# strasdat/ScaViSLAM

Hardware: AMD Instinct MI355X
Metric: stereo frames/sec + DWO Schur ms @ 50 KF / 20k pts (higher is better)
Workload: dtype u8/int32 (FAST, ZNSSD), f32+f64 (dense tracking), f64 (Schur); 1 GPU

## Files before the change

scavislam_amd/csrc/common.h:

```cpp
#pragma once
#include <hip/hip_runtime.h>
#include <stdint.h>
#include <stdio.h>
#include <memory>
#include <string>

#include "../../include/scavislam_hip.h"
#include "owned.h"
#include "devutil.h"

struct svs_ctx {
  int device = 0;
  int n_cu = 256;
  hipStream_t stream = nullptr;
  owned::Stream own_stream;
  owned::Event ev0, ev1;
  std::string err;
  DevBuf<void> scratch;
  DevBuf<void> match_scratch;
  int trk_nwg = 0;
  int trk_balance = 1;
  int trk_regs = 0;
  int full_nwg = 0;
  int match_legacy = 0;
  int mo_spec = 1;
  int fe_fuse_tail = 1;
  int match_order = 1;
  int fe_pipeline = 1;
  int fe_overlap = 1;
  int trk_seq_chi2 = 0;
  int trk_lazy_chi2 = 1;
  int trk_split = 10;
  int trk_cont_slots = 0;
  const double *match_src_T = nullptr, *match_src_Ta = nullptr;
  DevBuf<void> seq_buf;
  DevBuf<unsigned> seq_stats;
  owned::Event spin_ev;
  owned::Event lane_ev;
  bool spin_lane = false;
  int spin_demand = 0;
  long long spin_n_lane = 0, spin_n_gated = 0;
  long long stereo_n_prefilter16 = 0, stereo_n_prefilter4 = 0, stereo_n_strip_filter = 0, stereo_n_frame_filter = 0, stereo_n_validate_wide = 0, stereo_n_strips = 0;
  DevBuf<int> stereo_err;
  int xcd_swizzle = 1;
  float vocab_ms[3] = {0.f, 0.f, 0.f};
  int mo_legacy = 0;
  long long stereo_n_wide_search = 0;
};
int svs_spin_enter(svs_ctx *ctx, int n_workgroups = 0);
int svs_spin_leave(svs_ctx *ctx);
struct SvsSpinScope {
  svs_ctx *ctx; int rc; bool open;
  SvsSpinScope(svs_ctx *c, int n_workgroups = 0) : ctx(c), rc(svs_spin_enter(c, n_workgroups)), open(rc == 0) {}
  int leave() { if (!open) return SVS_OK; open = false; return svs_spin_leave(ctx); }
  ~SvsSpinScope() { if (open) (void)svs_spin_leave(ctx); }
  SvsSpinScope(const SvsSpinScope &) = delete;
  SvsSpinScope &operator=(const SvsSpinScope &) = delete;
};
int svs_ctx_grow(svs_ctx *ctx, DevBuf<void> svs_ctx::*which, size_t bytes, void **out);
inline int svs_ctx_scratch(svs_ctx *ctx, size_t bytes, void **out) { return svs_ctx_grow(ctx, &svs_ctx::scratch, bytes, out); }
inline int svs_ctx_match_scratch(svs_ctx *ctx, size_t bytes, void **out) { return svs_ctx_grow(ctx, &svs_ctx::match_scratch, bytes, out); }
size_t svs_dense_track_balance_bytes(int batch);
const int *svs_dense_track_balance_order(svs_ctx *ctx, void *d_bal_state, int batch);
int svs_dense_track_balance_init(svs_ctx *ctx, void *d_bal_state, int batch);
int svs_dense_track_cpu_sem_work(svs_ctx *ctx, const svs_dense_track_args *a, double *d_T_io, int32_t *d_passes_out, int batch, void *d_bal_state);
#define SVS_DEVICE(ctx) SVS_HIP(ctx, hipSetDevice((ctx)->device))

#define SVS_HIP(ctx, call)                                                              \
  do {                                                                                  \
    hipError_t e_ = (call);                                                             \
    if (e_ != hipSuccess) {                                                             \
      char buf_[512];                                                                   \
      snprintf(buf_, sizeof buf_, "%s:%d %s -> %s", __FILE__, __LINE__, #call,          \
               hipGetErrorString(e_));                                                  \
      (ctx)->err = buf_;                                                                \
      return SVS_ERR_HIP;                                                               \
    }                                                                                   \
  } while (0)

#define SVS_REQUIRE(ctx, cond)                                                          \
  do {                                                                                  \
    if (!(cond)) {                                                                      \
      char buf_[512];                                                                   \
      snprintf(buf_, sizeof buf_, "%s:%d requirement failed: %s", __FILE__, __LINE__,   \
               #cond);                                                                  \
      if (ctx) (ctx)->err = buf_;                                                       \
      return SVS_ERR_INVALID;                                                           \
    }                                                                                   \
  } while (0)

#define SVS_LAUNCH_CHECK(ctx) SVS_HIP(ctx, hipGetLastError())

int svs_pyr_down_u8_copy(svs_ctx *ctx, const uint8_t *d_src, int w, int h, int sstride, size_t s_bstride, uint8_t *d_dst, int dstride, size_t d_bstride,
                         uint8_t *d_copy, int cstride, size_t c_bstride, int batch);
struct svs_mo_tail {
  const svs_candidate_point *pts; size_t pts_b; const int32_t *n_new; float mre; svs_gated_point *gated; size_t gated_b; svs_point_stats *ptstats;
  const float *disp; int ds; size_t disp_b; svs_cam cams[3]; float *cloud[3]; size_t cloud_b[3];
  const int *order;
};
int svs_motion_only_gate_cloud(svs_ctx *ctx, const svs_match_result *d_results, int n, size_t res_bstride, const svs_cam *cam, const svs_pose_opt_params *prm,
                               double *d_T_io, svs_pose_opt_stats *d_stats, const svs_mo_tail *tail, int batch);
int svs_process_matched_points_dev(svs_ctx *ctx, const svs_match_result *d_results, const svs_candidate_point *d_pts, int n, size_t res_bstride,
                                   size_t pts_bstride, const int32_t *d_n_new_records, const svs_cam *cam, const double *d_T, float max_reproj_error,
                                   svs_gated_point *d_gated, size_t gated_bstride, svs_point_stats *d_stats, int batch);

int svs_pointcloud_cpu_sem_levels(svs_ctx *ctx, const float *d_disp, int disp_stride, size_t disp_bstride, const svs_cam *cams, const double *d_T, float *const *d_cloud,
                                  const size_t *cloud_bstride, int batch);

struct svs_loop;
int svs_loop_set_place_dev(svs_loop *l, int slot, int n, const float *d_desc, const double *d_uvu);
svs_ctx *svs_loop_ctx(svs_loop *l);
```

scavislam_amd/csrc/fast.hip:

```cpp
#include "common.h"
#include "fast_view.h"
#include <algorithm>
#include <cstdlib>
#include <vector>

namespace {

struct LevelDev {
  int w, h;
  int gx, gy, cell_w, cell_h;
  int min_inner, min_outer, max_inner, max_outer, fast_min, fast_max;
  int cell_base;
  uint32_t *bm;
  int bm_wpr, bm_stride;
  size_t bm_bstride;
  int16_t *xy;
};
struct FastParams {
  LevelDev lv[SVS_NUM_PYR_LEVELS];
  int n_levels, ncell_total, cap, t_lo;
  unsigned *hist;
  int *thr, *emit, *count, *offset;
  int *level_total;
  uint32_t *cand; int *cand_n;
  int *cell_tile0, *cell_ntile;
  int n_tiles;
  int swz;
};
constexpr int CAND_CAP = 2048;
constexpr int BM_LDS_MAX = 144 * 1024;
struct ImgPtrs {
  const uint8_t *img[SVS_NUM_PYR_LEVELS];
  int stride[SVS_NUM_PYR_LEVELS];
  size_t bstride[SVS_NUM_PYR_LEVELS];
};
struct TileDesc { int16_t level, cell, x0, y0; };

constexpr int TW = 64, TH = 32, HALO = 3;

__device__ __constant__ int8_t c_ring_dx[16] = {0, 1, 2, 3, 3, 3, 2, 1, 0, -1, -2, -3, -3, -3, -2, -1};
__device__ __constant__ int8_t c_ring_dy[16] = {3, 3, 2, 1, 0, -1, -2, -3, -3, -3, -2, -1, 0, 1, 2, 3};

__device__ __forceinline__ int arc9_maxmin(const int (&d)[16]) {
  int m2[16], m4[16], best = -1024;
#pragma unroll
  for (int k = 0; k < 16; ++k) m2[k] = min(d[k], d[(k + 1) & 15]);
#pragma unroll
  for (int k = 0; k < 16; ++k) m4[k] = min(m2[k], m2[(k + 2) & 15]);
#pragma unroll
  for (int k = 0; k < 16; ++k) {
    int m8 = min(m4[k], m4[(k + 4) & 15]);
    int m9 = min(m8, d[(k + 8) & 15]);
    best = max(best, m9);
  }
  return best;
}

typedef short s16x2 __attribute__((ext_vector_type(2)));
__device__ __forceinline__ s16x2 as_s16x2(uint32_t u) { s16x2 r; __builtin_memcpy(&r, &u, 4); return r; }
__device__ __forceinline__ s16x2 arc9_maxmin_pk(const s16x2 (&d)[16]) {
  s16x2 m2[16], m4[16], best = {-1024, -1024};
#pragma unroll
  for (int k = 0; k < 16; ++k) m2[k] = __builtin_elementwise_min(d[k], d[(k + 1) & 15]);
#pragma unroll
  for (int k = 0; k < 16; ++k) m4[k] = __builtin_elementwise_min(m2[k], m2[(k + 2) & 15]);
#pragma unroll
  for (int k = 0; k < 16; ++k) {
    const s16x2 m8 = __builtin_elementwise_min(m4[k], m4[(k + 4) & 15]);
    const s16x2 m9 = __builtin_elementwise_min(m8, d[(k + 8) & 15]);
    best = __builtin_elementwise_max(best, m9);
  }
  return best;
}

constexpr int LROW = 19;
__device__ __forceinline__ int byte_of(const uint32_t (&w)[3], int b) { return (w[b >> 2] >> (8 * (b & 3))) & 0xff; }
__device__ __forceinline__ uint32_t pair_of(const uint32_t (&w)[3], int b) {
  const int j = b >> 2, j1 = (j + 1 < 3) ? j + 1 : j;
  const unsigned i0 = (unsigned)(b & 3);
  const unsigned i1 = ((b + 1) >> 2) == j ? (unsigned)((b + 1) & 3) : 4u + (unsigned)((b + 1) & 3);
  return __builtin_amdgcn_perm(w[j1], w[j], i0 | (0x0cu << 8) | (i1 << 16) | (0x0cu << 24));
}

__global__ __launch_bounds__(256, 8) void fast_score_kernel(FastParams P, ImgPtrs I, const TileDesc *__restrict__ tiles) {
  __shared__ uint32_t s_img[(TH + 2 * HALO) * LROW];
  __shared__ unsigned s_hist[256];
  __shared__ uint16_t s_surv[TW * TH];
  __shared__ int s_ncorn, s_nsurv;
  unsigned wg = blockIdx.y * gridDim.x + blockIdx.x;
  if (P.swz) wg = xcd_contiguous(wg, gridDim.x * gridDim.y);
  const int tile_i = wg % gridDim.x, slot = wg / gridDim.x;
  const TileDesc td = tiles[tile_i];
  const LevelDev &L = P.lv[td.level];
  const int tid = threadIdx.x;
  const int ci = td.cell % L.gx, cj = td.cell / L.gx;
  const int u0 = ci * L.cell_w, v0 = cj * L.cell_h;
  const uint8_t *img = I.img[td.level] + (size_t)slot * I.bstride[td.level];
  const int istride = I.stride[td.level];
  s_hist[tid] = 0;
  const int gx0 = u0 + td.x0 - 4, gy0 = v0 + td.y0 - HALO;
  for (int i = tid; i < (TH + 2 * HALO) * 18; i += 256) {
    const int r = i / 18, c = i - r * 18;
    const int y = min(max(gy0 + r, 0), L.h - 1), x = gx0 + 4 * c;
    const uint8_t *row = img + (size_t)y * istride;
    const int xs = min(max(x, 0), L.w - 4), d = x - xs;
    uint32_t raw;
    __builtin_memcpy(&raw, row + xs, 4);
    const uint32_t v = d == 0 ? raw : d >= 4 || d <= -4 ? 0u : d > 0 ? raw >> (8 * d) : raw << (-8 * d);
    s_img[r * LROW + c] = v;
  }
  __syncthreads();
  const int tx = tid & 15;
  const int cx0 = td.x0 + 4 * tx;
  if (tid == 0) { s_ncorn = 0; s_nsurv = 0; }
  __syncthreads();
  const int t = P.t_lo;
  constexpr int RDX[16] = {0, 1, 2, 3, 3, 3, 2, 1, 0, -1, -2, -3, -3, -3, -2, -1};
  constexpr int RDY[16] = {3, 3, 2, 1, 0, -1, -2, -3, -3, -3, -2, -1, 0, 1, 2, 3};
#pragma unroll 1
  for (int ty = tid >> 4; ty < TH; ty += 16) {
    const int cy = td.y0 + ty;
    uint32_t win[7][3];
#pragma unroll
    for (int r = 0; r < 7; r += 3)
#pragma unroll
      for (int c = 0; c < 3; ++c) win[r][c] = s_img[(ty + r) * LROW + tx + c];
    const bool row_ok = cy >= 3 && cy < L.cell_h - 3;
    const uint32_t Kd = 0x7fff7fffu - (uint32_t)t * 0x00010001u;
#pragma unroll
    for (int p = 0; p < 2; ++p) {
      const uint32_t vpair = pair_of(win[3], 4 + 2 * p);
      const uint32_t Vd = vpair + Kd, Vb = Kd - vpair;
      uint32_t X[4], Y[4];
#pragma unroll
      for (int i = 0; i < 4; ++i) {
        const int q = 4 * i;
        const uint32_t rp = pair_of(win[3 + RDY[q]], 4 + 2 * p + RDX[q]);
        X[i] = Vd - rp; Y[i] = rp + Vb;
      }
      const uint32_t pass = ((X[0] & X[1]) | (X[1] & X[2]) | (X[2] & X[3]) | (X[3] & X[0]) | (Y[0] & Y[1]) | (Y[1] & Y[2]) | (Y[2] & Y[3]) | (Y[3] & Y[0])) & 0x80008000u;
#pragma unroll
      for (int h = 0; h < 2; ++h) {
        const int k = 2 * p + h, cx = cx0 + k;
        const bool surv = row_ok && cx >= 3 && cx < L.cell_w - 3 && ((pass >> (16 * h)) & 0x8000u) != 0;
        if (surv) { const int slot_i = atomicAdd(&s_nsurv, 1); s_surv[slot_i] = (uint16_t)((ty << 8) | (4 * tx + k)); }
      }
    }
  }
  __syncthreads();
  const int nsurv = s_nsurv;
  const uint8_t *s_b8 = reinterpret_cast<const uint8_t *>(s_img);
  uint32_t *cand = P.cand + ((size_t)slot * P.n_tiles + tile_i) * CAND_CAP;
  for (int i = tid; i < nsurv; i += 256) {
    const int code = s_surv[i], py = code >> 8, px = code & 0xff;
    const int cb = (py + 3) * (LROW * 4) + px + 4;
    const int v = s_b8[cb];
    s16x2 d[16];
#pragma unroll
    for (int q = 0; q < 16; ++q) {
      const int r = s_b8[cb + RDY[q] * (LROW * 4) + RDX[q]];
      const int x = v - r;
      d[q] = as_s16x2(((uint32_t)x & 0xffffu) | ((uint32_t)(-x) << 16));
    }
    const s16x2 b2 = arc9_maxmin_pk(d);
    const int sc = max((int)b2.x, (int)b2.y) - 1;
    if (sc >= t) {
      const int s8 = min(sc + 1, 255);
      atomicAdd(&s_hist[s8], 1u);
      cand[atomicAdd(&s_ncorn, 1)] = ((uint32_t)s8 << 24) | ((uint32_t)(td.y0 + py) << 12) | (uint32_t)(td.x0 + px);
    }
  }
  __syncthreads();
  if (tid == 0) P.cand_n[(size_t)slot * P.n_tiles + tile_i] = s_ncorn;
  const unsigned c = s_hist[tid];
  if (c) atomicAdd(&P.hist[((size_t)slot * P.ncell_total + L.cell_base + td.cell) * 256 + tid], c);
}

__global__ __launch_bounds__(256) void fast_adapt_kernel(FastParams P, int trials) {
  extern __shared__ int s_cnt[];
  const int slot = blockIdx.x;
  const int tid = threadIdx.x, lane = tid & 63, wave = tid >> 6;
  unsigned *hist = P.hist + (size_t)slot * P.ncell_total * 256;
  for (int c = wave; c < P.ncell_total; c += 4) {
    uint4 hv = *reinterpret_cast<const uint4 *>(hist + (size_t)c * 256 + 4 * lane);
    *reinterpret_cast<uint4 *>(hist + (size_t)c * 256 + 4 * lane) = make_uint4(0, 0, 0, 0);
    int a3 = hv.w, a2 = hv.z + a3, a1 = hv.y + a2, a0 = hv.x + a1;
    int tot = a0, run = tot;
#pragma unroll
    for (int o = 1; o < 64; o <<= 1) { int up = __shfl_down(run, o, 64); if (lane + o < 64) run += up; }
    int above = run - tot;
    s_cnt[c * 256 + 4 * lane + 0] = a0 + above;
    s_cnt[c * 256 + 4 * lane + 1] = a1 + above;
    s_cnt[c * 256 + 4 * lane + 2] = a2 + above;
    s_cnt[c * 256 + 4 * lane + 3] = a3 + above;
  }
  __syncthreads();
  int *thr = P.thr + (size_t)slot * P.ncell_total;
  int *emit = P.emit + (size_t)slot * P.ncell_total;
  int *count = P.count + (size_t)slot * P.ncell_total;
  int *offset = P.offset + (size_t)slot * P.ncell_total;
  int row = tid, lvl = -1, j = 0;
  for (int l = 0; l < P.n_levels; ++l) { if (row < P.lv[l].gy) { lvl = l; j = row; break; } row -= P.lv[l].gy; }
  if (lvl >= 0) {
    const LevelDev &L = P.lv[lvl];
    int prev_thr = -1, prev_prev_thr = -2;
    for (int i = 0; i < L.gx; ++i) {
      const int c = L.cell_base + j * L.gx + i;
      int t = thr[c], used = t, num = 0;
      if (trials <= 0) {
        int tc = min(max(t, 0), 255);
        num = tc + 1 <= 255 ? s_cnt[c * 256 + tc + 1] : 0;
      }
      for (int trial = 0; trial < trials; ++trial) {
        used = t;
        int tc = min(max(t, 0), 255);
        num = tc + 1 <= 255 ? s_cnt[c * 256 + tc + 1] : 0;
        if (prev_prev_thr == t) { t = (t + prev_prev_thr) / 2; break; }
        prev_prev_thr = prev_thr;
        prev_thr = t;
        if (num < L.min_inner) {
          if (t <= L.fast_min) break;
          --t;
          if (num < L.min_outer) { if (t <= L.fast_min) break; --t; continue; }
        } else if (num > L.max_inner) {
          if (t >= L.fast_max) break;
          ++t;
          if (num > L.max_outer) { if (t >= L.fast_max) break; ++t; continue; }
        }
        break;
      }
      thr[c] = t; emit[c] = used; count[c] = num;
    }
  }
  __syncthreads();
  if (tid < P.n_levels) {
    const LevelDev &L = P.lv[tid];
    int run = 0;
    for (int c = L.cell_base; c < L.cell_base + L.gx * L.gy; ++c) { offset[c] = run; run += count[c]; }
    P.level_total[(size_t)slot * P.n_levels + tid] = run;
  }
}

template <int NT>
__global__ __launch_bounds__(NT) void fast_compact_bitmap_kernel(FastParams P) {
  extern __shared__ uint32_t s_bm[];
  const int slot = blockIdx.y, c = blockIdx.x, tid = threadIdx.x, lane = tid & 63, wave = tid >> 6;
  int lvl = 0;
  while (lvl + 1 < P.n_levels && c >= P.lv[lvl + 1].cell_base) ++lvl;
  const LevelDev &L = P.lv[lvl];
  const int cl = c - L.cell_base, ci = cl % L.gx, cj = cl / L.gx;
  const int u0 = ci * L.cell_w, v0 = cj * L.cell_h;
  const int rows = L.cell_h, wpr = L.bm_wpr;
  int *s_row = reinterpret_cast<int *>(s_bm + rows * wpr);
  const int thr1 = min(max(P.emit[(size_t)slot * P.ncell_total + c], 0), 255) + 1;
  const int base = P.offset[(size_t)slot * P.ncell_total + c];
  for (int i = tid; i < rows * wpr; i += NT) s_bm[i] = 0u;
  __syncthreads();
  if (thr1 <= 255) {
    const int t0 = P.cell_tile0[c], nt = P.cell_ntile[c];
    for (int t = wave; t < nt; t += NT / 64) {
      const int n = min(P.cand_n[(size_t)slot * P.n_tiles + t0 + t], CAND_CAP);
      const uint32_t *cand = P.cand + ((size_t)slot * P.n_tiles + t0 + t) * CAND_CAP;
      for (int i = lane; i < n; i += 64) {
        const uint32_t r = cand[i];
        if ((int)(r >> 24) >= thr1) {
          const int x = r & 0xfffu, y = (r >> 12) & 0xfffu;
          atomicOr(&s_bm[y * wpr + (x >> 5)], 1u << (x & 31));
        }
      }
    }
  }
  __syncthreads();
  for (int r = tid; r < rows; r += NT) {
    int n = 0;
    for (int j = 0; j < wpr; ++j) n += __popc(s_bm[r * wpr + j]);
    s_row[r] = n;
  }
  __syncthreads();
  if (wave == 0) {
    int carry = 0;
    for (int r0 = 0; r0 < rows; r0 += 64) {
      const int v = r0 + lane < rows ? s_row[r0 + lane] : 0;
      int run = v;
#pragma unroll
      for (int o = 1; o < 64; o <<= 1) { const int dn = __shfl_up(run, o, 64); if (lane >= o) run += dn; }
      if (r0 + lane < rows) s_row[r0 + lane] = carry + run - v;
      carry += __shfl(run, 63, 64);
    }
  }
  __syncthreads();
  int16_t *xy = L.xy + (size_t)slot * P.cap * 2;
  uint32_t *gbm = L.bm + (size_t)slot * (L.bm_bstride / 4) + (size_t)v0 * (L.bm_stride / 4) + ci * wpr;
  for (int i = tid; i < rows * wpr; i += NT) {
    const int r = i / wpr, j = i - r * wpr;
    uint32_t w = s_bm[i];
    gbm[(size_t)r * (L.bm_stride / 4) + j] = w;
    if (w) {
      int pos = base + s_row[r];
      for (int k = 0; k < j; ++k) pos += __popc(s_bm[r * wpr + k]);
      while (w) {
        const int b = __ffs((int)w) - 1;
        w &= w - 1;
        if (pos < P.cap) {
          const uint32_t pk = (uint32_t)(uint16_t)(u0 + 32 * j + b) | ((uint32_t)(uint16_t)(v0 + r) << 16);
          __builtin_memcpy(xy + 2 * pos, &pk, 4);
        }
        ++pos;
      }
    }
  }
}

}

struct svs_fast {
  svs_ctx *ctx;
  FastParams P;
  int batch;
  TileDesc *d_tiles; int n_tiles;
  DevBuf<uint32_t> bm[SVS_NUM_PYR_LEVELS], cand;
  DevBuf<int16_t> xy[SVS_NUM_PYR_LEVELS];
  DevBuf<unsigned> hist;
  DevBuf<int> thr, emit, count, offset, level_total, cand_n, cell_tile0, cell_ntile;
  DevBuf<TileDesc> tiles;
  ~svs_fast() { (void)hipStreamSynchronize(ctx->stream); }
  size_t cmp_lds = 0;
};

extern "C" int svs_fast_create(svs_ctx *ctx, int n_levels, const int32_t *w, const int32_t *h,
                               const svs_fastgrid *grids, int batch, int cap, svs_fast **out) {
  SVS_REQUIRE(ctx, ctx && out && w && h && grids && n_levels >= 1 && n_levels <= SVS_NUM_PYR_LEVELS && batch >= 1 && cap >= 1);
  SVS_DEVICE(ctx);
  {
    int nc = 0;
    for (int l = 0; l < n_levels; ++l) {
      const svs_fastgrid &g = grids[l];
      SVS_REQUIRE(ctx, g.gx >= 1 && g.gy >= 1 && g.gx * g.gy <= SVS_MAX_CELLS && g.cell_w >= 1 && g.cell_h >= 1 && g.cell_w * g.gx <= w[l] && g.cell_h * g.gy <= h[l]);
      SVS_REQUIRE(ctx, g.cell_w <= 4096 && g.cell_h <= 4096);
      SVS_REQUIRE(ctx, ((size_t)g.cell_h * ((g.cell_w + 31) / 32) + g.cell_h) * 4 <= (size_t)BM_LDS_MAX);
      nc += g.gx * g.gy;
    }
    SVS_REQUIRE(ctx, (size_t)nc * 256 * 4 <= 64 * 1024);
  }
  std::unique_ptr<svs_fast> f(new svs_fast());
  f->ctx = ctx; f->batch = batch;
  FastParams &P = f->P;
  P = FastParams{};
  P.n_levels = n_levels; P.cap = cap;
  std::vector<TileDesc> tiles;
  std::vector<int> cell_tile0, cell_ntile;
  int cell_base = 0, t_lo = 255;
  for (int l = 0; l < n_levels; ++l) {
    const svs_fastgrid &g = grids[l];
    LevelDev &L = P.lv[l];
    L.w = w[l]; L.h = h[l]; L.gx = g.gx; L.gy = g.gy; L.cell_w = g.cell_w; L.cell_h = g.cell_h;
    L.min_inner = g.min_inner; L.min_outer = g.min_outer; L.max_inner = g.max_inner; L.max_outer = g.max_outer;
    L.fast_min = g.fast_min; L.fast_max = g.fast_max; L.cell_base = cell_base;
    L.bm_wpr = (g.cell_w + 31) / 32;
    const int gap = 32 * L.bm_wpr - g.cell_w;
    L.bm_stride = ((std::max(w[l], g.gx * g.cell_w) + gap * (g.gx - 1) + 7) / 8 + 8 + 15) / 16 * 16;
    SVS_REQUIRE(ctx, L.bm_stride >= 4 * L.bm_wpr * g.gx);
    L.bm_bstride = (size_t)L.bm_stride * h[l] + 16;
    SVS_HIP(ctx, f->bm[l].alloc_bytes(L.bm_bstride * batch, &L.bm));
    SVS_HIP(ctx, hipMemsetAsync(L.bm, 0, L.bm_bstride * batch, ctx->stream));
    f->cmp_lds = std::max(f->cmp_lds, ((size_t)g.cell_h * L.bm_wpr + g.cell_h) * 4);
    SVS_HIP(ctx, f->xy[l].alloc(2 * (size_t)cap * batch, &L.xy));
    for (int c = 0; c < g.gx * g.gy; ++c) {
      t_lo = std::min(t_lo, std::min(g.fast_min, g.thr[c]));
      cell_tile0.push_back((int)tiles.size());
      for (int y0 = 0; y0 < g.cell_h; y0 += TH)
        for (int x0 = 0; x0 < g.cell_w; x0 += TW) tiles.push_back(TileDesc{(int16_t)l, (int16_t)c, (int16_t)x0, (int16_t)y0});
      cell_ntile.push_back((int)tiles.size() - cell_tile0.back());
    }
    cell_base += g.gx * g.gy;
  }
  P.ncell_total = cell_base;
  P.t_lo = std::max(t_lo, 0);
  if (f->cmp_lds > 64 * 1024) {
    SVS_HIP(ctx, hipFuncSetAttribute(reinterpret_cast<const void *>(&fast_compact_bitmap_kernel<256>), hipFuncAttributeMaxDynamicSharedMemorySize, (int)f->cmp_lds));
    SVS_HIP(ctx, hipFuncSetAttribute(reinterpret_cast<const void *>(&fast_compact_bitmap_kernel<1024>), hipFuncAttributeMaxDynamicSharedMemorySize, (int)f->cmp_lds));
  }
  size_t nc = (size_t)P.ncell_total * batch;
  SVS_HIP(ctx, f->hist.alloc(nc * 256, &P.hist));
  SVS_HIP(ctx, hipMemsetAsync(P.hist, 0, nc * 256 * sizeof(unsigned), ctx->stream));
  SVS_HIP(ctx, f->thr.alloc(nc, &P.thr));
  SVS_HIP(ctx, f->emit.alloc(nc, &P.emit));
  SVS_HIP(ctx, f->count.alloc(nc, &P.count));
  SVS_HIP(ctx, f->offset.alloc(nc, &P.offset));
  SVS_HIP(ctx, f->level_total.alloc((size_t)batch * n_levels, &P.level_total));
  SVS_HIP(ctx, hipMemsetAsync(P.emit, 0, nc * sizeof(int), ctx->stream));
  SVS_HIP(ctx, hipMemsetAsync(P.count, 0, nc * sizeof(int), ctx->stream));
  SVS_HIP(ctx, hipMemsetAsync(P.offset, 0, nc * sizeof(int), ctx->stream));
  SVS_HIP(ctx, hipMemsetAsync(P.level_total, 0, (size_t)batch * n_levels * sizeof(int), ctx->stream));
  std::vector<int> thr0(nc);
  for (int b = 0; b < batch; ++b)
    for (int l = 0; l < n_levels; ++l)
      for (int c = 0; c < grids[l].gx * grids[l].gy; ++c) thr0[(size_t)b * P.ncell_total + P.lv[l].cell_base + c] = grids[l].thr[c];
  SVS_HIP(ctx, hipMemcpyAsync(P.thr, thr0.data(), nc * sizeof(int), hipMemcpyHostToDevice, ctx->stream));
  f->n_tiles = (int)tiles.size();
  P.n_tiles = f->n_tiles;
  SVS_HIP(ctx, f->cand.alloc((size_t)batch * tiles.size() * CAND_CAP, &P.cand));
  SVS_HIP(ctx, f->cand_n.alloc((size_t)batch * tiles.size(), &P.cand_n));
  SVS_HIP(ctx, f->cell_tile0.alloc(cell_tile0.size(), &P.cell_tile0));
  SVS_HIP(ctx, f->cell_ntile.alloc(cell_ntile.size(), &P.cell_ntile));
  SVS_HIP(ctx, hipMemcpyAsync(P.cell_tile0, cell_tile0.data(), sizeof(int) * cell_tile0.size(), hipMemcpyHostToDevice, ctx->stream));
  SVS_HIP(ctx, hipMemcpyAsync(P.cell_ntile, cell_ntile.data(), sizeof(int) * cell_ntile.size(), hipMemcpyHostToDevice, ctx->stream));
  SVS_HIP(ctx, f->tiles.alloc(tiles.size(), &f->d_tiles));
  SVS_HIP(ctx, hipMemcpyAsync(f->d_tiles, tiles.data(), sizeof(TileDesc) * tiles.size(), hipMemcpyHostToDevice, ctx->stream));
  SVS_HIP(ctx, hipStreamSynchronize(ctx->stream));
  *out = f.release();
  return SVS_OK;
}

extern "C" int svs_fast_destroy(svs_fast *f) {
  if (!f) return SVS_OK;
  delete f;
  return SVS_OK;
}

extern "C" int svs_fast_detect(svs_fast *f, const uint8_t *const *d_img, const int32_t *stride, const size_t *bstride,
                               int n_batch, int trials) {
  SVS_REQUIRE(f ? f->ctx : nullptr, f && d_img && stride && bstride && n_batch >= 1 && n_batch <= f->batch && trials >= 0);
  SVS_DEVICE(f->ctx);
  svs_ctx *ctx = f->ctx;
  ImgPtrs I{};
  for (int l = 0; l < f->P.n_levels; ++l) { I.img[l] = d_img[l]; I.stride[l] = stride[l]; I.bstride[l] = bstride[l]; }
  f->P.swz = ctx->xcd_swizzle;
  hipLaunchKernelGGL(fast_score_kernel, dim3(f->n_tiles, n_batch), dim3(256), 0, ctx->stream, f->P, I, f->d_tiles);
  SVS_LAUNCH_CHECK(ctx);
  hipLaunchKernelGGL(fast_adapt_kernel, dim3(n_batch), dim3(256), (size_t)f->P.ncell_total * 256 * sizeof(int), ctx->stream, f->P, trials);
  SVS_LAUNCH_CHECK(ctx);
  if ((long)f->P.ncell_total * n_batch <= 1024) hipLaunchKernelGGL(fast_compact_bitmap_kernel<1024>, dim3(f->P.ncell_total, n_batch), dim3(1024), f->cmp_lds, ctx->stream, f->P);
  else hipLaunchKernelGGL(fast_compact_bitmap_kernel<256>, dim3(f->P.ncell_total, n_batch), dim3(256), f->cmp_lds, ctx->stream, f->P);
  SVS_LAUNCH_CHECK(ctx);
  return SVS_OK;
}

extern "C" int svs_fast_download(svs_fast *f, int slot, int level, int16_t *h_xy, int cap, int32_t *h_n,
                                 int32_t *h_cell_count, int32_t *h_emit_thr, int32_t *h_thr_state) {
  SVS_REQUIRE(f ? f->ctx : nullptr, f && slot >= 0 && slot < f->batch && level >= 0 && level < f->P.n_levels);
  SVS_DEVICE(f->ctx);
  svs_ctx *ctx = f->ctx;
  const FastParams &P = f->P;
  const LevelDev &L = P.lv[level];
  int total = 0;
  SVS_HIP(ctx, hipMemcpyAsync(&total, P.level_total + (size_t)slot * P.n_levels + level, sizeof(int), hipMemcpyDeviceToHost, ctx->stream));
  SVS_HIP(ctx, hipStreamSynchronize(ctx->stream));
  if (h_n) *h_n = total;
  int nc = L.gx * L.gy;
  size_t co = (size_t)slot * P.ncell_total + L.cell_base;
  if (h_cell_count) SVS_HIP(ctx, hipMemcpyAsync(h_cell_count, P.count + co, nc * sizeof(int), hipMemcpyDeviceToHost, ctx->stream));
  if (h_emit_thr) SVS_HIP(ctx, hipMemcpyAsync(h_emit_thr, P.emit + co, nc * sizeof(int), hipMemcpyDeviceToHost, ctx->stream));
  if (h_thr_state) SVS_HIP(ctx, hipMemcpyAsync(h_thr_state, P.thr + co, nc * sizeof(int), hipMemcpyDeviceToHost, ctx->stream));
  int ncopy = std::min(std::min(total, cap), P.cap);
  if (h_xy && ncopy > 0)
    SVS_HIP(ctx, hipMemcpyAsync(h_xy, L.xy + (size_t)slot * P.cap * 2, sizeof(int16_t) * 2 * (size_t)ncopy, hipMemcpyDeviceToHost, ctx->stream));
  SVS_HIP(ctx, hipStreamSynchronize(ctx->stream));
  if (h_xy && (total > cap || total > P.cap)) return SVS_ERR_CAPACITY;
  return SVS_OK;
}

extern "C" int svs_fast_set_thresholds(svs_fast *f, int slot, int level, const int32_t *h_thr) {
  SVS_REQUIRE(f ? f->ctx : nullptr, f && h_thr && slot >= 0 && slot < f->batch && level >= 0 && level < f->P.n_levels);
  SVS_DEVICE(f->ctx);
  svs_ctx *ctx = f->ctx;
  const LevelDev &L = f->P.lv[level];
  int nc = L.gx * L.gy;
  for (int c = 0; c < nc; ++c) SVS_REQUIRE(ctx, h_thr[c] >= f->P.t_lo);
  SVS_HIP(ctx, hipMemcpyAsync(f->P.thr + (size_t)slot * f->P.ncell_total + L.cell_base, h_thr, nc * sizeof(int), hipMemcpyHostToDevice, ctx->stream));
  SVS_HIP(ctx, hipStreamSynchronize(ctx->stream));
  return SVS_OK;
}

extern "C" int svs_fast_device_view(svs_fast *f, int level, const uint32_t **d_corner_bits, int32_t *row_stride_bytes, size_t *batch_stride_bytes,
                                    int32_t *cell_column_bits, const int32_t **d_emit_thr, size_t *emit_bstride) {
  SVS_REQUIRE(f ? f->ctx : nullptr, f && level >= 0 && level < f->P.n_levels);
  const LevelDev &L = f->P.lv[level];
  if (d_corner_bits) *d_corner_bits = L.bm;
  if (row_stride_bytes) *row_stride_bytes = L.bm_stride;
  if (batch_stride_bytes) *batch_stride_bytes = L.bm_bstride;
  if (cell_column_bits) *cell_column_bits = 32 * L.bm_wpr;
  if (d_emit_thr) *d_emit_thr = f->P.emit + L.cell_base;
  if (emit_bstride) *emit_bstride = (size_t)f->P.ncell_total;
  return SVS_OK;
}

FastView svs_fast_view_internal(const svs_fast *f) {
  FastView v{};
  v.n_levels = f->P.n_levels; v.emit = f->P.emit; v.ncell_total = f->P.ncell_total;
  for (int l = 0; l < f->P.n_levels; ++l) {
    const LevelDev &L = f->P.lv[l];
    v.bm[l] = reinterpret_cast<const uint8_t *>(L.bm); v.bm_stride[l] = L.bm_stride; v.bm_bstride[l] = L.bm_bstride; v.bm_gap[l] = 32 * L.bm_wpr - L.cell_w;
    v.cell_base[l] = L.cell_base; v.gx[l] = L.gx; v.gy[l] = L.gy; v.cell_w[l] = L.cell_w; v.cell_h[l] = L.cell_h;
    v.w[l] = L.w; v.h[l] = L.h;
  }
  return v;
}

FastThrView svs_fast_thr_view_internal(svs_fast *f) {
  FastThrView v{};
  v.thr = f->P.thr; v.ncell_total = f->P.ncell_total; v.t_lo = f->P.t_lo; v.n_levels = f->P.n_levels; v.batch = f->batch;
  for (int l = 0; l < f->P.n_levels; ++l) { v.cell_base[l] = f->P.lv[l].cell_base; v.ncell[l] = f->P.lv[l].gx * f->P.lv[l].gy; }
  return v;
}

FastListView svs_fast_list_view_internal(const svs_fast *f) {
  FastListView v{};
  v.n_levels = f->P.n_levels; v.batch = f->batch; v.cap = f->P.cap; v.level_total = f->P.level_total; v.count = f->P.count; v.ncell_total = f->P.ncell_total;
  for (int l = 0; l < f->P.n_levels; ++l) { v.xy[l] = f->P.lv[l].xy; v.cell_base[l] = f->P.lv[l].cell_base; v.ncell[l] = f->P.lv[l].gx * f->P.lv[l].gy; }
  return v;
}
```

scavislam_amd/csrc/image.hip:

```cpp
#include "common.h"
#include <algorithm>
#include <mutex>
#include <vector>
#include <stdlib.h>

namespace {
struct SpinLane { svs_ctx *c; hipEvent_t ev; int cus; };
struct SpinGate { std::mutex m; hipEvent_t last = nullptr; svs_ctx *owner = nullptr; int last_cus = 0; std::vector<SpinLane> lanes; };
SpinGate g_spin_gate[64];
SpinGate &gate_of(const svs_ctx *c) { return g_spin_gate[(unsigned)c->device % 64u]; }
}
constexpr int SVS_SPIN_SMALL = 16;
int svs_spin_enter(svs_ctx *c, int n_workgroups) {
  SpinGate &g = gate_of(c);
  const int demand = n_workgroups > 0 ? std::min(n_workgroups, c->n_cu) : c->n_cu;
  g.m.lock();
  for (size_t i = 0; i < g.lanes.size();) {
    if (g.lanes[i].c != c && hipEventQuery(g.lanes[i].ev) == hipErrorNotReady) ++i;
    else if (g.lanes[i].c == c) ++i;
    else { g.lanes[i] = g.lanes.back(); g.lanes.pop_back(); }
  }
  int lanes_busy = 0;
  for (const SpinLane &l : g.lanes) if (l.c != c) lanes_busy += l.cus;
  const bool gated_busy = g.last && g.owner != c && hipEventQuery(g.last) == hipErrorNotReady;
  (void)hipGetLastError();
  c->spin_demand = demand;
  c->spin_lane = n_workgroups > 0 && n_workgroups <= SVS_SPIN_SMALL && demand + lanes_busy + (gated_busy ? g.last_cus : 0) <= c->n_cu;
  if (c->spin_lane) { ++c->spin_n_lane; return SVS_OK; }
  ++c->spin_n_gated;
  hipError_t e = hipSuccess;
  if (g.last && g.owner != c) e = hipStreamWaitEvent(c->stream, g.last, 0);
  if (demand + lanes_busy > c->n_cu)
    for (const SpinLane &l : g.lanes) if (l.c != c && e == hipSuccess) e = hipStreamWaitEvent(c->stream, l.ev, 0);
  if (e != hipSuccess) { g.m.unlock(); c->err = std::string("svs_spin_enter: hipStreamWaitEvent -> ") + hipGetErrorString(e); return SVS_ERR_HIP; }
  return SVS_OK;
}
int svs_spin_leave(svs_ctx *c) {
  SpinGate &g = gate_of(c);
  hipError_t e = hipSuccess;
  owned::Event &ev = c->spin_lane ? c->lane_ev : c->spin_ev;
  if (!ev) e = ev.create(hipEventDisableTiming);
  if (e == hipSuccess) e = hipEventRecord(ev, c->stream);
  if (e == hipSuccess) {
    if (c->spin_lane) {
      bool found = false;
      for (SpinLane &l : g.lanes) if (l.c == c) { l.ev = ev; l.cus = c->spin_demand; found = true; }
      if (!found) g.lanes.push_back(SpinLane{c, ev, c->spin_demand});
    } else { g.last = ev; g.owner = c; g.last_cus = c->spin_demand; }
  }
  c->spin_lane = false;
  g.m.unlock();
  if (e != hipSuccess) { c->err = std::string("svs_spin_leave: ") + hipGetErrorString(e); return SVS_ERR_HIP; }
  return SVS_OK;
}
static void spin_forget(svs_ctx *c) {
  SpinGate &g = gate_of(c);
  std::lock_guard<std::mutex> lk(g.m);
  for (size_t i = 0; i < g.lanes.size();) { if (g.lanes[i].c == c) { g.lanes[i] = g.lanes.back(); g.lanes.pop_back(); } else ++i; }
  if (g.owner == c) { g.last = nullptr; g.owner = nullptr; g.last_cus = 0; }
}
extern "C" int svs_ctx_create(int device, void *hip_stream, svs_ctx **out) {
  if (!out) return SVS_ERR_INVALID;
  int n = 0;
  if (hipGetDeviceCount(&n) != hipSuccess || n <= 0 || device < 0 || device >= n) return SVS_ERR_NO_DEVICE;
  std::unique_ptr<svs_ctx> c(new svs_ctx());
  c->device = device;
  if (hipSetDevice(device) != hipSuccess) return SVS_ERR_NO_DEVICE;
  { int cu = 0; if (hipDeviceGetAttribute(&cu, hipDeviceAttributeMultiprocessorCount, device) == hipSuccess && cu > 0) c->n_cu = cu; }
  if (hip_stream) c->stream = (hipStream_t)hip_stream;
  else if (c->own_stream.create(hipStreamNonBlocking) != hipSuccess) return SVS_ERR_HIP;
  else c->stream = c->own_stream;
  if (c->ev0.create() != hipSuccess || c->ev1.create() != hipSuccess) return SVS_ERR_HIP;
  if (c->stereo_err.alloc(32) != hipSuccess || hipMemset(c->stereo_err, 0, 32 * sizeof(int)) != hipSuccess) return SVS_ERR_HIP;
  auto env_int = [](const char *name, int lo, int hi) { const char *e = getenv(name); if (!e) return 0; const int v = atoi(e); return v < lo ? lo : (v > hi ? hi : v); };
  c->trk_nwg = env_int("SVS_TRK_NWG", 1, 64);
  if (const char *e = getenv("SVS_TRK_BALANCE")) { const int v = atoi(e); c->trk_balance = v < 0 || v > 1 ? 1 : v; }
  c->trk_regs = getenv("SVS_TRK_ONE_PER_CU") ? 1 : (getenv("SVS_TRK_TWO_PER_CU") ? 2 : 0);
  c->full_nwg = env_int("SVS_FULL_NWG", 1, 1024);
  *out = c.release();
  return SVS_OK;
}
extern "C" int svs_ctx_destroy(svs_ctx *c) {
  if (!c) return SVS_OK;
  (void)hipStreamSynchronize(c->stream);
  spin_forget(c);
  delete c;
  return SVS_OK;
}
int svs_ctx_grow(svs_ctx *c, DevBuf<void> svs_ctx::*which, size_t bytes, void **out) {
  SVS_REQUIRE(c, c && out);
  DevBuf<void> &buf = c->*which;
  if (buf.bytes() < bytes) {
    SVS_DEVICE(c);
    if (buf) SVS_HIP(c, hipStreamSynchronize(c->stream));
    SVS_HIP(c, buf.reserve(bytes, bytes + bytes / 2 + 4096));
  }
  *out = buf;
  return SVS_OK;
}
extern "C" int svs_ctx_set_option(svs_ctx *c, const char *name, int value) {
  SVS_REQUIRE(c, c && name && value >= 0);
  const std::string n(name);
  if (n == "trk_nwg") c->trk_nwg = value > 64 ? 64 : value;
  else if (n == "trk_regs") c->trk_regs = value > 2 ? 0 : value;
  else if (n == "trk_balance") c->trk_balance = value > 1 ? 1 : value;
  else if (n == "full_nwg") c->full_nwg = value > 1024 ? 1024 : value;
  else if (n == "mo_legacy") c->mo_legacy = value != 0;
  else if (n == "match_legacy") c->match_legacy = (int)value;
  else if (n == "fe_overlap") c->fe_overlap = value != 0;
  else if (n == "fe_pipeline") c->fe_pipeline = value != 0;
  else if (n == "match_order") c->match_order = value != 0;
  else if (n == "fe_fuse_tail") c->fe_fuse_tail = value != 0;
  else if (n == "mo_spec") c->mo_spec = value != 0;
  else if (n == "xcd_swizzle") c->xcd_swizzle = value != 0;
  else if (n == "trk_split") c->trk_split = value > 15 ? 15 : value;
  else if (n == "trk_cont_slots") c->trk_cont_slots = value > 4096 ? 4096 : value;
  else if (n == "trk_seq_chi2") c->trk_seq_chi2 = value != 0;
  else if (n == "trk_lazy_chi2") c->trk_lazy_chi2 = value > 2 ? 1 : value;
  else SVS_REQUIRE(c, !"unknown option");
  return SVS_OK;
}
extern "C" int svs_ctx_get_stat(svs_ctx *c, const char *name, long long *out) {
  SVS_REQUIRE(c, c && name && out);
  const std::string n(name);
  if (n == "spin_lane_launches") { *out = c->spin_n_lane; return SVS_OK; }
  if (n == "spin_gated_launches") { *out = c->spin_n_gated; return SVS_OK; }
  if (n == "live_device_bytes") { *out = owned::g_live_device_bytes; return SVS_OK; }
  if (n == "live_pinned_bytes") { *out = owned::g_live_pinned_bytes; return SVS_OK; }
  if (n == "live_sync_objects") { *out = owned::g_live_sync_objects; return SVS_OK; }
  if (n == "stereo_prefilter16_calls") { *out = c->stereo_n_prefilter16; return SVS_OK; }
  if (n == "stereo_prefilter4_calls") { *out = c->stereo_n_prefilter4; return SVS_OK; }
  if (n == "stereo_strip_filter_calls") { *out = c->stereo_n_strip_filter; return SVS_OK; }
  if (n == "stereo_strip_filter_strips") { *out = c->stereo_n_strips; return SVS_OK; }
  if (n == "stereo_frame_filter_calls") { *out = c->stereo_n_frame_filter; return SVS_OK; }
  if (n == "stereo_validate_wide_calls") { *out = c->stereo_n_validate_wide; return SVS_OK; }
  if (n == "stereo_wide_search_calls") { *out = c->stereo_n_wide_search; return SVS_OK; }
  if (n == "stereo_speckle_error_mask") {
    int m = 0;
    SVS_DEVICE(c);
    SVS_HIP(c, hipMemcpyAsync(&m, c->stereo_err, sizeof m, hipMemcpyDeviceToHost, c->stream));
    SVS_HIP(c, hipStreamSynchronize(c->stream));
    *out = m;
    return SVS_OK;
  }
  SVS_REQUIRE(c, n == "trk_exact_sums" || n == "trk_exact_fallbacks");
  unsigned v[2] = {0, 0};
  if (c->seq_stats) {
    SVS_DEVICE(c);
    SVS_HIP(c, hipMemcpyAsync(v, c->seq_stats, sizeof v, hipMemcpyDeviceToHost, c->stream));
    SVS_HIP(c, hipStreamSynchronize(c->stream));
  }
  *out = n == "trk_exact_sums" ? v[0] : v[1];
  return SVS_OK;
}
extern "C" int svs_api_version(void) { return SVS_API_VERSION; }
extern "C" void svs_pose_opt_params_default(svs_pose_opt_params *p) {
  if (!p) return;
  __builtin_memset(p, 0, sizeof *p);
  p->robust_kernel = 1; p->num_iter = 15; p->kernel_param = 2.0; p->initial_mu = -1.0; p->tau = 1e-5; p->min_obs = 0;
}
extern "C" int svs_ctx_sync(svs_ctx *c) { SVS_REQUIRE(c, c); SVS_HIP(c, hipStreamSynchronize(c->stream)); return SVS_OK; }
extern "C" void *svs_ctx_stream(svs_ctx *c) { return c ? (void *)c->stream : nullptr; }
extern "C" const char *svs_last_error(svs_ctx *c) { return c ? c->err.c_str() : "null ctx"; }
extern "C" int svs_malloc(svs_ctx *c, size_t bytes, void **p) {
  SVS_REQUIRE(c, c && p);
  SVS_HIP(c, hipSetDevice(c->device));
  SVS_HIP(c, owned::caller_malloc(p, bytes ? bytes : 1));
  return SVS_OK;
}
extern "C" int svs_free(svs_ctx *c, void *p) { SVS_REQUIRE(c, c); if (p) SVS_HIP(c, owned::caller_free(p)); return SVS_OK; }
extern "C" int svs_memcpy_h2d(svs_ctx *c, void *d, const void *h, size_t n) {
  SVS_REQUIRE(c, c);
  SVS_DEVICE(c);
  SVS_HIP(c, hipMemcpyAsync(d, h, n, hipMemcpyHostToDevice, c->stream));
  SVS_HIP(c, hipStreamSynchronize(c->stream));
  return SVS_OK;
}
extern "C" int svs_memcpy_d2h(svs_ctx *c, void *h, const void *d, size_t n) {
  SVS_REQUIRE(c, c);
  SVS_DEVICE(c);
  SVS_HIP(c, hipMemcpyAsync(h, d, n, hipMemcpyDeviceToHost, c->stream));
  SVS_HIP(c, hipStreamSynchronize(c->stream));
  return SVS_OK;
}
extern "C" int svs_timer_start(svs_ctx *c) { SVS_REQUIRE(c, c);
  SVS_DEVICE(c); SVS_HIP(c, hipEventRecord(c->ev0, c->stream)); return SVS_OK; }
extern "C" int svs_timer_stop_ms(svs_ctx *c, float *ms) {
  SVS_REQUIRE(c, c && ms);
  SVS_DEVICE(c);
  SVS_HIP(c, hipEventRecord(c->ev1, c->stream));
  SVS_HIP(c, hipEventSynchronize(c->ev1));
  SVS_HIP(c, hipEventElapsedTime(ms, c->ev0, c->ev1));
  return SVS_OK;
}

template <bool COPY>
__global__ __launch_bounds__(256) void pyr_down_u8_kernel(const uint8_t *__restrict__ src, int w, int h, int ss,
                                                         size_t sb, uint8_t *__restrict__ dst, int dw, int dh,
                                                         int ds, size_t db, uint8_t *__restrict__ cpy, int cs, size_t cb, int swz) {
  unsigned wg = blockIdx.y * gridDim.x + blockIdx.x;
  if (swz) wg = xcd_contiguous(wg, gridDim.x * gridDim.y);
  const int ncol = (dw + 3) >> 2, nrow = (dh + 1) >> 1;
  const int bz = wg / gridDim.x, item = (int)(wg % gridDim.x) * 256 + (int)threadIdx.x;
  if (item >= ncol * nrow) return;
  const int oyh = item / ncol;
  const int ox = 4 * (item - oyh * ncol), oy = 2 * oyh;
  src += (size_t)bz * sb;
  dst += (size_t)bz * db;
  if (COPY) cpy += (size_t)bz * cb;
  const int sx0 = 2 * ox - 2, sy0 = 2 * oy - 2;
  const bool left = sx0 < 0, cross2 = sx0 + 12 > w;
  const bool fast = w >= 16 && sx0 + 8 <= w;
  uint32_t sel0 = 0x03020100u, sel2 = 0x03020100u;
  int off2 = sx0 + 8;
  if (left) sel0 = 0x01000102u;
  if (cross2) {
    off2 = w - 4;
    sel2 = 0;
#pragma unroll
    for (int k = 0; k < 4; ++k) {
      const int c = sx0 + 8 + k, cr = c < w ? c : 2 * w - 2 - c;
      sel2 |= (uint32_t)max(min(cr - (w - 4), 3), 0) << (8 * k);
    }
  }
  typedef unsigned short us2_t __attribute__((ext_vector_type(2)));
  union Pk2 { uint32_t u; us2_t h; };
  Pk2 hp[7][2];
  const uint32_t W4 = 1u | (4u << 8) | (6u << 16) | (4u << 24);
  uint32_t D0[7], D1[7], D2[7];
  if (h >= 8 && __all(fast)) {
#pragma unroll
    for (int r = 0; r < 7; ++r) {
      int y = sy0 + r;
      y = y < 0 ? -y : y;
      y = y >= h ? 2 * h - 2 - y : y;
      const uint8_t *p = src + (size_t)y * ss;
      D0[r] = ld_unaligned<uint32_t>(p + (left ? 0 : sx0)); D1[r] = ld_unaligned<uint32_t>(p + sx0 + 4); D2[r] = ld_unaligned<uint32_t>(p + off2);
    }
  } else {
#pragma unroll 1
    for (int r = 0; r < 7; ++r) {
      const uint8_t *p = src + (size_t)reflect101(sy0 + r, h) * ss;
      uint32_t d0, d1, d2;
      if (fast) {
        d0 = __builtin_amdgcn_perm(0u, ld_unaligned<uint32_t>(p + (left ? 0 : sx0)), sel0);
        d1 = ld_unaligned<uint32_t>(p + sx0 + 4);
        d2 = __builtin_amdgcn_perm(0u, ld_unaligned<uint32_t>(p + off2), sel2);
      } else {
        uint32_t bt[12];
#pragma unroll
        for (int k = 0; k < 11; ++k) bt[k] = p[reflect101(sx0 + k, w)];
        bt[11] = 0;
        d0 = bt[0] | (bt[1] << 8) | (bt[2] << 16) | (bt[3] << 24);
        d1 = bt[4] | (bt[5] << 8) | (bt[6] << 16) | (bt[7] << 24);
        d2 = bt[8] | (bt[9] << 8) | (bt[10] << 16);
      }
      if (r == 0) { D0[0] = d0; D1[0] = d1; D2[0] = d2; } else if (r == 1) { D0[1] = d0; D1[1] = d1; D2[1] = d2; } else if (r == 2) { D0[2] = d0; D1[2] = d1; D2[2] = d2; }
      else if (r == 3) { D0[3] = d0; D1[3] = d1; D2[3] = d2; } else if (r == 4) { D0[4] = d0; D1[4] = d1; D2[4] = d2; } else if (r == 5) { D0[5] = d0; D1[5] = d1; D2[5] = d2; }
      else { D0[6] = d0; D1[6] = d1; D2[6] = d2; }
    }
    sel0 = 0x03020100u; sel2 = 0x03020100u;
  }
#pragma unroll
  for (int r = 0; r < 7; ++r) {
    const uint32_t d0 = __builtin_amdgcn_perm(0u, D0[r], sel0), d1 = D1[r], d2 = __builtin_amdgcn_perm(0u, D2[r], sel2);
    const uint32_t d01 = __builtin_amdgcn_alignbyte(d1, d0, 2);
    const uint32_t d12 = __builtin_amdgcn_alignbyte(d2, d1, 2);
    const uint32_t h0 = __builtin_amdgcn_udot4(d0, W4, d1 & 0xffu, false);
    const uint32_t h1 = __builtin_amdgcn_udot4(d01, W4, d12 & 0xffu, false);
    const uint32_t h2 = __builtin_amdgcn_udot4(d1, W4, d2 & 0xffu, false);
    const uint32_t h3 = __builtin_amdgcn_udot4(d12, W4, (d2 >> 16) & 0xffu, false);
    hp[r][0].u = h0 | (h1 << 16);
    hp[r][1].u = h2 | (h3 << 16);
    if (COPY && r >= 2 && r <= 5) {
      const int cy = 2 * oy + r - 2, cx = 2 * ox;
      if (cy < h) {
        uint8_t *q = cpy + (size_t)cy * cs + cx;
        if (cx + 7 < w && (cs & 3) == 0 && (cb & 3) == 0 && ((uintptr_t)cpy & 3) == 0) {
          reinterpret_cast<uint32_t *>(q)[0] = d01;
          reinterpret_cast<uint32_t *>(q)[1] = d12;
        } else {
#pragma unroll
          for (int j = 0; j < 8; ++j) if (cx + j < w) q[j] = (uint8_t)((j < 4 ? d01 : d12) >> (8 * (j & 3)));
        }
      }
    }
  }
  const us2_t c4 = {4, 4}, c6 = {6, 6}, c128 = {128, 128};
#pragma unroll
  for (int o = 0; o < 2; ++o) {
    if (oy + o >= dh) break;
    uint32_t v[4];
#pragma unroll
    for (int q = 0; q < 2; ++q) {
      const us2_t acc = (hp[2 * o][q].h + hp[2 * o + 4][q].h) + c4 * (hp[2 * o + 1][q].h + hp[2 * o + 3][q].h) + c6 * hp[2 * o + 2][q].h;
      Pk2 t;
      t.h = acc;
      v[2 * q] = ((t.u & 0xffffu) + 128u) >> 8;
      v[2 * q + 1] = ((t.u >> 16) + 128u) >> 8;
    }
    (void)c128;
    const uint32_t packed = v[0] | (v[1] << 8) | (v[2] << 16) | (v[3] << 24);
    uint8_t *q = dst + (size_t)(oy + o) * ds + ox;
    if (ox + 3 < dw && ((ds | (int)(db & 3)) & 3) == 0 && ((uintptr_t)dst & 3) == 0) *reinterpret_cast<uint32_t *>(q) = packed;
    else {
#pragma unroll
      for (int j = 0; j < 4; ++j) if (ox + j < dw) q[j] = (uint8_t)v[j];
    }
  }
}

extern "C" int svs_pyr_down_u8(svs_ctx *ctx, const uint8_t *d_src, int w, int h, int sstride, size_t s_bstride,
                               uint8_t *d_dst, int dstride, size_t d_bstride, int batch) {
  SVS_REQUIRE(ctx, ctx && d_src && d_dst && w >= 3 && h >= 3 && batch >= 1);
  SVS_DEVICE(ctx);
  int dw = (w + 1) / 2, dh = (h + 1) / 2;
  dim3 grid(div_up(div_up(dw, 4) * div_up(dh, 2), 256), batch), block(256);
  hipLaunchKernelGGL(pyr_down_u8_kernel<false>, grid, block, 0, ctx->stream, d_src, w, h, sstride, s_bstride, d_dst, dw,
                     dh, dstride, d_bstride, (uint8_t *)nullptr, 0, (size_t)0, ctx->xcd_swizzle);
  SVS_LAUNCH_CHECK(ctx);
  return SVS_OK;
}
int svs_pyr_down_u8_copy(svs_ctx *ctx, const uint8_t *d_src, int w, int h, int sstride, size_t s_bstride, uint8_t *d_dst, int dstride, size_t d_bstride,
                         uint8_t *d_copy, int cstride, size_t c_bstride, int batch) {
  SVS_REQUIRE(ctx, ctx && d_src && d_dst && d_copy && w >= 3 && h >= 3 && batch >= 1);
  SVS_DEVICE(ctx);
  int dw = (w + 1) / 2, dh = (h + 1) / 2;
  dim3 grid(div_up(div_up(dw, 4) * div_up(dh, 2), 256), batch), block(256);
  hipLaunchKernelGGL(pyr_down_u8_kernel<true>, grid, block, 0, ctx->stream, d_src, w, h, sstride, s_bstride, d_dst, dw, dh, dstride, d_bstride, d_copy,
                     cstride, c_bstride, ctx->xcd_swizzle);
  SVS_LAUNCH_CHECK(ctx);
  return SVS_OK;
}

__global__ __launch_bounds__(256) void convert_sobel_kernel(const uint8_t *__restrict__ src, int w, int h, int ss,
                                                            size_t sb, float *__restrict__ img, float *__restrict__ dx,
                                                            float *__restrict__ dy, int fs, size_t fb) {
  const float sc = (float)(1. / 255.);
  int x4 = (blockIdx.x * blockDim.x + threadIdx.x) * 4;
  int y = blockIdx.y;
  if (x4 >= w) return;
  src += (size_t)blockIdx.z * sb;
  size_t fo = (size_t)blockIdx.z * fb + (size_t)y * fs;
  const uint8_t *row = src + (size_t)y * ss;
  const uint8_t *rowm = src + (size_t)reflect101(y - 1, h) * ss;
  const uint8_t *rowp = src + (size_t)reflect101(y + 1, h) * ss;
  float c[6];
#pragma unroll
  for (int k = 0; k < 6; ++k) c[k] = (float)row[reflect101(x4 - 1 + k, w)] * sc;
  if (x4 + 3 < w && (fs & 3) == 0 && (fb & 3) == 0 && (((uintptr_t)img | (uintptr_t)dx | (uintptr_t)dy) & 15) == 0) {
    float4 vi = make_float4(c[1], c[2], c[3], c[4]);
    float4 vx = make_float4(c[2] - c[0], c[3] - c[1], c[4] - c[2], c[5] - c[3]);
    float4 vy;
    vy.x = (float)rowp[x4] * sc - (float)rowm[x4] * sc;
    vy.y = (float)rowp[x4 + 1] * sc - (float)rowm[x4 + 1] * sc;
    vy.z = (float)rowp[x4 + 2] * sc - (float)rowm[x4 + 2] * sc;
    vy.w = (float)rowp[x4 + 3] * sc - (float)rowm[x4 + 3] * sc;
    *reinterpret_cast<float4 *>(img + fo + x4) = vi;
    *reinterpret_cast<float4 *>(dx + fo + x4) = vx;
    *reinterpret_cast<float4 *>(dy + fo + x4) = vy;
    return;
  }
#pragma unroll
  for (int k = 0; k < 4; ++k) {
    int x = x4 + k;
    if (x < w) {
      img[fo + x] = c[k + 1];
      dx[fo + x] = c[k + 2] - c[k];
      dy[fo + x] = (float)rowp[x] * sc - (float)rowm[x] * sc;
    }
  }
}

extern "C" int svs_convert_sobel_f32(svs_ctx *ctx, const uint8_t *d_src, int w, int h, int sstride, size_t s_bstride,
                                     float *d_img, float *d_dx, float *d_dy, int fstride, size_t f_bstride,
                                     int batch) {
  SVS_REQUIRE(ctx, ctx && d_src && d_img && d_dx && d_dy && w >= 2 && h >= 2 && batch >= 1);
  SVS_DEVICE(ctx);
  dim3 block(64), grid(div_up(div_up(w, 4), 64), h, batch);
  hipLaunchKernelGGL(convert_sobel_kernel, grid, block, 0, ctx->stream, d_src, w, h, sstride, s_bstride, d_img,
                     d_dx, d_dy, fstride, f_bstride);
  SVS_LAUNCH_CHECK(ctx);
  return SVS_OK;
}
```

Before: 224,700 frames/s.

## Raise per-cell FAST threshold floor and aggregate LDS atomics per wavefront

The FAST score kernel now derives its detection threshold from the cell's current adaptive threshold minus a margin that depends on the trial count, instead of always using the global low threshold. This prunes candidates that the adaptation step could never select, cutting scoring, histogram and candidate-write work. It also replaces per-lane LDS atomics for survivor and corner compaction with one wavefront ballot, prefix count and a single atomic per wave. The floor relies on the margin being wide enough to keep adaptive selection unchanged, and it can be turned off with a new option.

```diff
diff --git a/scavislam_amd/csrc/common.h b/scavislam_amd/csrc/common.h
--- a/scavislam_amd/csrc/common.h
+++ b/scavislam_amd/csrc/common.h
@@ -26,6 +26,7 @@
   int mo_spec = 1;
   int fe_fuse_tail = 1;
   int match_order = 1;
+  int fast_floor = 1;
   int fe_pipeline = 1;
   int fe_overlap = 1;
   int trk_seq_chi2 = 0;
diff --git a/scavislam_amd/csrc/fast.hip b/scavislam_amd/csrc/fast.hip
--- a/scavislam_amd/csrc/fast.hip
+++ b/scavislam_amd/csrc/fast.hip
@@ -26,6 +26,7 @@
   int *cell_tile0, *cell_ntile;
   int n_tiles;
   int swz;
+  int floor;
 };
 constexpr int CAND_CAP = 2048;
 constexpr int BM_LDS_MAX = 144 * 1024;
@@ -82,7 +83,9 @@
   return __builtin_amdgcn_perm(w[j1], w[j], i0 | (0x0cu << 8) | (i1 << 16) | (0x0cu << 24));
 }
 
-__global__ __launch_bounds__(256, 8) void fast_score_kernel(FastParams P, ImgPtrs I, const TileDesc *__restrict__ tiles) {
+__device__ __forceinline__ int lanes_below(unsigned long long bal) { return (int)__builtin_amdgcn_mbcnt_hi((uint32_t)(bal >> 32), __builtin_amdgcn_mbcnt_lo((uint32_t)bal, 0u)); }
+
+__global__ __launch_bounds__(256, 8) void fast_score_kernel(FastParams P, ImgPtrs I, const TileDesc *__restrict__ tiles, int trials) {
   __shared__ uint32_t s_img[(TH + 2 * HALO) * LROW];
   __shared__ unsigned s_hist[256];
   __shared__ uint16_t s_surv[TW * TH];
@@ -97,6 +100,7 @@
   const int u0 = ci * L.cell_w, v0 = cj * L.cell_h;
   const uint8_t *img = I.img[td.level] + (size_t)slot * I.bstride[td.level];
   const int istride = I.stride[td.level];
+  const int thr_c = P.thr[(size_t)slot * P.ncell_total + L.cell_base + td.cell];
   s_hist[tid] = 0;
   const int gx0 = u0 + td.x0 - 4, gy0 = v0 + td.y0 - HALO;
   for (int i = tid; i < (TH + 2 * HALO) * 18; i += 256) {
@@ -114,7 +118,7 @@
   const int cx0 = td.x0 + 4 * tx;
   if (tid == 0) { s_ncorn = 0; s_nsurv = 0; }
   __syncthreads();
-  const int t = P.t_lo;
+  const int t = P.floor ? min(max(P.t_lo, thr_c - 2 * min(max(trials - 1, 0), 128)), 255) : P.t_lo;
   constexpr int RDX[16] = {0, 1, 2, 3, 3, 3, 2, 1, 0, -1, -2, -3, -3, -3, -2, -1};
   constexpr int RDY[16] = {3, 3, 2, 1, 0, -1, -2, -3, -3, -3, -2, -1, 0, 1, 2, 3};
 #pragma unroll 1
@@ -127,6 +131,7 @@
       for (int c = 0; c < 3; ++c) win[r][c] = s_img[(ty + r) * LROW + tx + c];
     const bool row_ok = cy >= 3 && cy < L.cell_h - 3;
     const uint32_t Kd = 0x7fff7fffu - (uint32_t)t * 0x00010001u;
+    bool surv[4];
 #pragma unroll
     for (int p = 0; p < 2; ++p) {
       const uint32_t vpair = pair_of(win[3], 4 + 2 * p);
@@ -142,33 +147,53 @@
 #pragma unroll
       for (int h = 0; h < 2; ++h) {
         const int k = 2 * p + h, cx = cx0 + k;
-        const bool surv = row_ok && cx >= 3 && cx < L.cell_w - 3 && ((pass >> (16 * h)) & 0x8000u) != 0;
-        if (surv) { const int slot_i = atomicAdd(&s_nsurv, 1); s_surv[slot_i] = (uint16_t)((ty << 8) | (4 * tx + k)); }
-      }
-    }
+        surv[k] = row_ok && cx >= 3 && cx < L.cell_w - 3 && ((pass >> (16 * h)) & 0x8000u) != 0;
+      }
+    }
+    unsigned long long bal[4];
+    int n_wave = 0, at[4];
+#pragma unroll
+    for (int k = 0; k < 4; ++k) { bal[k] = __ballot(surv[k]); at[k] = n_wave + lanes_below(bal[k]); n_wave += __popcll(bal[k]); }
+    int base = 0;
+    if ((tid & 63) == 0 && n_wave) base = atomicAdd(&s_nsurv, n_wave);
+    base = __builtin_amdgcn_readfirstlane(base);
+#pragma unroll
+    for (int k = 0; k < 4; ++k)
+      if (surv[k]) s_surv[base + at[k]] = (uint16_t)((ty << 8) | (4 * tx + k));
   }
   __syncthreads();
   const int nsurv = s_nsurv;
   const uint8_t *s_b8 = reinterpret_cast<const uint8_t *>(s_img);
   uint32_t *cand = P.cand + ((size_t)slot * P.n_tiles + tile_i) * CAND_CAP;
-  for (int i = tid; i < nsurv; i += 256) {
-    const int code = s_surv[i], py = code >> 8, px = code & 0xff;
-    const int cb = (py + 3) * (LROW * 4) + px + 4;
-    const int v = s_b8[cb];
-    s16x2 d[16];
-#pragma unroll
-    for (int q = 0; q < 16; ++q) {
-      const int r = s_b8[cb + RDY[q] * (LROW * 4) + RDX[q]];
-      const int x = v - r;
-      d[q] = as_s16x2(((uint32_t)x & 0xffffu) | ((uint32_t)(-x) << 16));
-    }
-    const s16x2 b2 = arc9_maxmin_pk(d);
-    const int sc = max((int)b2.x, (int)b2.y) - 1;
-    if (sc >= t) {
-      const int s8 = min(sc + 1, 255);
-      atomicAdd(&s_hist[s8], 1u);
-      cand[atomicAdd(&s_ncorn, 1)] = ((uint32_t)s8 << 24) | ((uint32_t)(td.y0 + py) << 12) | (uint32_t)(td.x0 + px);
-    }
+  for (int i0 = 0; i0 < nsurv; i0 += 256) {
+    const int i = i0 + tid;
+    bool corner = false;
+    uint32_t rec = 0;
+    if (i < nsurv) {
+      const int code = s_surv[i], py = code >> 8, px = code & 0xff;
+      const int cb = (py + 3) * (LROW * 4) + px + 4;
+      const int v = s_b8[cb];
+      s16x2 d[16];
+#pragma unroll
+      for (int q = 0; q < 16; ++q) {
+        const int r = s_b8[cb + RDY[q] * (LROW * 4) + RDX[q]];
+        const int x = v - r;
+        d[q] = as_s16x2(((uint32_t)x & 0xffffu) | ((uint32_t)(-x) << 16));
+      }
+      const s16x2 b2 = arc9_maxmin_pk(d);
+      const int sc = max((int)b2.x, (int)b2.y) - 1;
+      if (sc >= t) {
+        const int s8 = min(sc + 1, 255);
+        atomicAdd(&s_hist[s8], 1u);
+        corner = true;
+        rec = ((uint32_t)s8 << 24) | ((uint32_t)(td.y0 + py) << 12) | (uint32_t)(td.x0 + px);
+      }
+    }
+    const unsigned long long bal = __ballot(corner);
+    int base = 0;
+    if ((tid & 63) == 0 && bal) base = atomicAdd(&s_ncorn, __popcll(bal));
+    base = __builtin_amdgcn_readfirstlane(base);
+    if (corner) cand[base + lanes_below(bal)] = rec;
   }
   __syncthreads();
   if (tid == 0) P.cand_n[(size_t)slot * P.n_tiles + tile_i] = s_ncorn;
@@ -426,7 +451,8 @@
   ImgPtrs I{};
   for (int l = 0; l < f->P.n_levels; ++l) { I.img[l] = d_img[l]; I.stride[l] = stride[l]; I.bstride[l] = bstride[l]; }
   f->P.swz = ctx->xcd_swizzle;
-  hipLaunchKernelGGL(fast_score_kernel, dim3(f->n_tiles, n_batch), dim3(256), 0, ctx->stream, f->P, I, f->d_tiles);
+  f->P.floor = ctx->fast_floor;
+  hipLaunchKernelGGL(fast_score_kernel, dim3(f->n_tiles, n_batch), dim3(256), 0, ctx->stream, f->P, I, f->d_tiles, trials);
   SVS_LAUNCH_CHECK(ctx);
   hipLaunchKernelGGL(fast_adapt_kernel, dim3(n_batch), dim3(256), (size_t)f->P.ncell_total * 256 * sizeof(int), ctx->stream, f->P, trials);
   SVS_LAUNCH_CHECK(ctx);
diff --git a/scavislam_amd/csrc/image.hip b/scavislam_amd/csrc/image.hip
--- a/scavislam_amd/csrc/image.hip
+++ b/scavislam_amd/csrc/image.hip
@@ -111,6 +111,7 @@
   else if (n == "fe_pipeline") c->fe_pipeline = value != 0;
   else if (n == "match_order") c->match_order = value != 0;
   else if (n == "fe_fuse_tail") c->fe_fuse_tail = value != 0;
+  else if (n == "fast_floor") c->fast_floor = value != 0;
   else if (n == "mo_spec") c->mo_spec = value != 0;
   else if (n == "xcd_swizzle") c->xcd_swizzle = value != 0;
   else if (n == "trk_split") c->trk_split = value > 15 ? 15 : value;
```

New measurement: 232,200 frames/s, median of 6. 3.3% higher.
